# acproject/wsi-segmentation-pipeline

Hardware: AMD Instinct MI355X
Metric: patches/sec (256×256×3) whole-slide inference, 1/2/4/8 MI355X + CPU ref (higher is better)
Workload: dtype fp16 + MX-fp6 cross terms (fp32 accumulate); 1 GPU; cfg3: ONE 40000x40000 synthetic slide, tile 256 stride 256 -> 24648 tiles sharded over 1 rank(s) (each holds only its own slide regions: 4.80 GB on rank 0), ResNet-18 trunk + Classifier, fused read+normalise+conv HIP path, 1 all-gather, float64 stitch + softmax; tiles_total=24648, batch=6200, mode=mx, parallelism=tile-shard x1 + 1 all-gather, batches_in_flight=2

## Files before the change

include/wsi_hip.h:

```cpp
#ifndef WSI_HIP_H
#define WSI_HIP_H
#include <stddef.h>
#include <stdint.h>

#ifdef __cplusplus
extern "C" {
#endif

#define WSI_HIP_ABI_VERSION 9
int wsi_hip_abi_version(void);

size_t wsi_pf_bytes(int n, int h, int w, int c, int planes);
long long wsi_pf_pixel_index(int n, int y, int x, int h, int w);

size_t wsi_prepack_conv_bytes(int cout, int cin, int k, int planes);
int wsi_prepack_conv(const float* w, const float* bn_weight, const float* bn_bias, const float* bn_mean,
                     const float* bn_var, float eps, int cout, int cin, int k, int planes, void* wpk_out,
                     float* bias_out);
size_t wsi_prepack_stem_bytes(int planes);
int wsi_prepack_stem(const float* w, const float* bn_weight, const float* bn_bias, const float* bn_mean,
                     const float* bn_var, float eps, int planes, void* wpk_out, float* bias_out);
int wsi_prepack_stem_u8(const float* w, const float* bn_weight, const float* bn_bias, const float* bn_mean,
                        const float* bn_var, float eps, const float mean[3], const float std_[3], int planes,
                        void* wpk_out, float* bias_out);
// ... 14 lines not shown

enum {
    WSI_STEM_MODE_UNFUSED = 0,
    WSI_STEM_MODE_FUSED = 1,
    WSI_STEM_MODE_FUSED_LUT = 2,
    WSI_STEM_MODE_FUSED_ONE_STRIP = 3,
    WSI_STEM_MODE_FUSED_STRIPS = 4
};
int wsi_stem_set_mode(int fused, int rows_per_seg);

int wsi_conv3x3_bn_act(const void* in_pf, void* out_pf, const void* resid_pf, const void* wpk, const float* bias,
                       int n, int h_in, int w_in, int cin, int cout, int stride, int relu, int planes,
                       void* stream);
int wsi_conv1x1_bn(const void* in_pf, void* out_pf, const void* wpk, const float* bias, int n, int h_in, int w_in,
                   int cin, int cout, int stride, int planes, void* stream);
int wsi_conv1x1_bn_act(const void* in_pf, void* out_pf, const void* resid_pf, const void* wpk, const float* bias,
                       int n, int h_in, int w_in, int cin, int cout, int stride, int relu, int planes, void* stream);
int wsi_conv3x3_up_concat_bn_act(const void* up_pf, const void* skip_pf, void* out_pf, const void* wpk, const float* bias, int n, int h, int w,
                                 int c_up, int c_skip, int cout, int relu, int planes, void* stream);
int wsi_conv3x3s2_ds_fused(const void* in_pf, void* out_conv_pf, void* out_ds_pf, const void* wpk3, const float* bias3,
                           const void* wpk1, const float* bias1, int n, int h_in, int w_in, int cin, int cout, int planes,
                           void* stream);
int wsi_s2_slab_images(int n, int h_in, int w_in, int cin, int planes);
size_t wsi_pf_split_bytes(int n, int h, int w, int c, int planes);
int wsi_conv3x3_bn_act_split(const void* in_pf, void* out_split, const void* resid_pf, const void* wpk, const float* bias,
                             int n, int h, int w, int cin, int cout, int relu, int planes, void* stream);
int wsi_conv3x3s2_ds_fused_split(const void* in_split, void* out_conv_pf, void* out_ds_pf, const void* wpk3,
                                 const float* bias3, const void* wpk1, const float* bias1, int n, int h_in, int w_in,
                                 int cin, int cout, int planes, void* stream);
enum {
    WSI_CONV_MODE_S2_GATHER = 0,
    WSI_CONV_MODE_S2_SLAB = 1,
    WSI_CONV_MODE_S2_SLAB_128 = 3,
    WSI_CONV_MODE_XCD_ORDER = 8,
    WSI_CONV_MODE_WIDE_FROM_256 = 16,
    WSI_CONV_MODE_WIDE_NEVER = 32,
    WSI_CONV_MODE_S2_ABLATE = 64,
    WSI_CONV_MODE_NO_S2_SPLIT = 128,
    WSI_CONV_MODE_XCD_RANGES_OFF = 256,
    WSI_CONV_MODE_XCD_RANGES_L1 = 512,
    WSI_CONV_MODE_L1_SLAB3 = 1024,
    WSI_CONV_MODE_NO_DS_FOLD = 2048,
    WSI_CONV_MODE_NO_SLAB_PAIR = 4096,
    WSI_CONV_MODE_EPILOGUE_PIECES = 8192,
    WSI_CONV_MODE_L1_LINES128 = 16384,
    WSI_CONV_MODE_S2_NT2 = 32768,
    WSI_CONV_MODE_UNET_CONCAT_PASS = 65536,
    WSI_CONV_MODE_WIDE_NO_D8 = 131072,
    WSI_CONV_MODE_PW_GATHER = 262144,
    WSI_CONV_MODE_L1_PERSISTENT = 1048576,
    WSI_CONV_MODE_UNET_NO_TAIL = 2097152,
    WSI_CONV_MODE_UNET_TAIL_FORM1 = 4194304,
    WSI_CONV_MODE_UNET_X0_UNFUSED = 8388608,
    WSI_CONV_MODE_LINKNET_NO_TAIL = 16777216
};
int wsi_conv_set_mode(int mode);
int wsi_conv3x3_bn_act_cfg(const void* in_pf, void* out_pf, const void* resid_pf, const void* wpk, const float* bias,
                           int n, int h_in, int w_in, int cin, int cout, int stride, int relu, int planes, int cfg,
                           void* stream);

int wsi_avgpool_fc(const void* in_pf, int n, int h, int w, int c, const float* fc_w, const float* fc_b, int k,
                   float* feat_out, float* logits_out, int planes, void* stream);
int wsi_linear(const float* x, const float* w, const float* bias, float* y, int b, int k, int j, int relu,
               void* stream);

int wsi_pf_pack(const float* in_nchw, void* out_pf, int n, int c, int h, int w, int planes, void* stream);
int wsi_pf_unpack(const void* in_pf, float* out_nchw, int n, int c, int h, int w, int planes, void* stream);

#define WSI_TRUNK_MAX_BLOCKS 36
typedef struct {
    const void* stem_w;   const float* stem_b;
    const void* stem_w_u8; const float* stem_b_u8;
    float norm[6];
    int blocks[4];
    const void* conv_w[2 * WSI_TRUNK_MAX_BLOCKS]; const float* conv_b[2 * WSI_TRUNK_MAX_BLOCKS];
    const void* down_w[3];  const float* down_b[3];
    const float* head_w;  const float* head_b;  int head_k;
    int planes;
} wsi_trunk_weights;

size_t wsi_trunk_workspace_bytes(int n, int h, int w, int planes);
int wsi_trunk_workspace_init(void* workspace, int n, int h, int w, int planes, void* stream);
int wsi_trunk_workspace_release(void* workspace);
int wsi_trunk_forward(const wsi_trunk_weights* wt, const float* in_f32, const uint8_t* slide,
                      long long slide_pitch_bytes, int slide_h, int slide_w, const int* tile_xy, const float* lut,
                      int n, int h, int w, void* workspace, int workspace_n, float* feat_out ,
                      float* logits_out , float* fmap_out ,
                      void* stream);
int wsi_trunk_set_chunks(int stem_chunk, int layer1_chunk);
int wsi_trunk_forward_tap(const wsi_trunk_weights* wt, const float* in_f32, const uint8_t* slide,
                          long long slide_pitch_bytes, int slide_h, int slide_w, const int* tile_xy, const float* lut,
                          int n, int h, int w, void* workspace, int workspace_n, int stop_after, float* tap_out_nchw,
                          void* stream);

typedef struct {
    const void* stem_w;   const float* stem_b;
    const void* stem_w_u8; const float* stem_b_u8;
    float norm[6];
    int blocks[4];
    const void* conv_w[3 * WSI_TRUNK_MAX_BLOCKS]; const float* conv_b[3 * WSI_TRUNK_MAX_BLOCKS];
    const void* down_w[4];  const float* down_b[4];
    const float* head_w;  const float* head_b;  int head_k;
    int planes;
} wsi_bneck_weights;
size_t wsi_bneck_workspace_bytes(int n, int h, int w, int planes);
int wsi_bneck_workspace_init(void* workspace, int n, int h, int w, int planes, void* stream);
// ... 304 lines not shown
```

wsi_segmentation_pipeline_amd/csrc/capi.hip:

```cpp
#include "internal.h"
#include "edt_dev.h"
#include "regions_dev.h"
#include "../../include/wsi_hip.h"

ConvRoutes g_routes;

StemArgs stem_args(const TileSource& src, const void* wpk, const float* bias, float* scratch, int n, int h, int w) {
    StemArgs a;
    a.mode = src.in_f32 ? 0 : 1;
    a.in_f32 = src.in_f32; a.slide = src.slide; a.slide_pitch = src.pitch; a.SH = src.SH; a.SW = src.SW;
    a.origins = src.tile_xy; a.lut = src.lut; a.wpk = wpk; a.bias = bias; a.out = scratch;
    a.N = n; a.H = h; a.W = w; a.wpk_u8 = nullptr; a.bias_u8 = nullptr;
    return a;
}

int stem_run(const TileSource& src, const void* stem_wpk, const float* stem_bias, const void* stem_wpk_u8, const float* stem_bias_u8,
             const float* norm_mean_std, int n, int h, int w, float* scratch, void* out_pf, int planes, void* stream, int out96,
             long long plane96, void* x0_pf) {
    if (!stem_wpk || !stem_bias || !scratch || !out_pf || n <= 0 || h % 16 || w % 4) return WSI_EINVAL;
    if (!src.valid()) return WSI_EINVAL;
    StemArgs a = stem_args(src, stem_wpk, stem_bias, scratch, n, h, w);
    if (stem_wpk_u8 && stem_bias_u8 && norm_mean_std && !src.in_f32 && g_routes.stem_u8x) { a.wpk_u8 = stem_wpk_u8; a.bias_u8 = stem_bias_u8; }
    if (out96 && planes != 3) return WSI_EINVAL;
    if (x0_pf && !(a.wpk_u8 && g_routes.stem_fused && planes == 2)) return WSI_EINVAL;
// ... 201 lines not shown
int wsi_conv3x3s2_ds_fused(const void* in_pf, void* out_conv_pf, void* out_ds_pf, const void* wpk3, const float* bias3,
                           const void* wpk1, const float* bias1, int n, int h_in, int w_in, int cin, int cout, int planes,
                           void* stream) {
    if (!s2_ds_ok(in_pf, out_conv_pf, out_ds_pf, wpk3, bias3, wpk1, bias1, n, h_in, w_in, false)) return WSI_EINVAL;
    ConvArgs a = s2_ds_args(in_pf, out_conv_pf, out_ds_pf, wpk3, bias3, wpk1, bias1, n, h_in, w_in, cin, cout);
    const int per = wsi_s2_slab_images(n, h_in, w_in, cin, planes);
    const size_t bpc = planes == 1 ? PFmt<1>::BPC : PFmt<2>::BPC;
    const size_t in_img = (size_t)(h_in + 1) * (w_in + 1) * cin * bpc, out_img = (size_t)(h_in / 2 + 1) * (w_in / 2 + 1) * cout * bpc;
    int rc = WSI_EINVAL;
    for (int n0 = 0; per > 0 && n0 < n; n0 += per) {
        const int nn = n - n0 < per ? n - n0 : per;
        a.in = (const char*)in_pf + n0 * in_img;
        a.out = (char*)out_conv_pf + n0 * out_img;
        a.out2 = (char*)out_ds_pf + n0 * out_img;
        a.gi = pf_geom_fd(nn, h_in, w_in, cin);
        a.go = pf_geom_fd(nn, h_in / 2, w_in / 2, cout);
        rc = wsi_s2_dispatch(a, planes, (hipStream_t)stream);
        if (rc) break;
    }
    if (rc == WSI_EINVAL) {
        ConvCall c = {.in = in_pf, .out = out_conv_pf, .wpk = wpk3, .bias = bias3, .n = n, .h = h_in, .w = w_in, .cin = cin, .cout = cout,
                      .stride = 2, .ksize = 3, .relu = 1, .planes = planes, .stream = stream, .cfg = 0};
        rc = conv_common(c);
        c.out = out_ds_pf; c.wpk = wpk1; c.bias = bias1; c.ksize = 1; c.relu = 0;
        if (!rc) rc = conv_common(c);
    }
    return rc;
}

int wsi_conv_set_mode(int mode) {
    ConvRoutes& r = g_routes;
    const int base = mode & 7;
    r.s2_slab = base != WSI_CONV_MODE_S2_GATHER;
    r.s2_small_tiles = base != WSI_CONV_MODE_S2_SLAB_128;
    r.xcd_order = (mode & WSI_CONV_MODE_XCD_ORDER) ? 1 : 0;
    r.wide_min_c = (mode & WSI_CONV_MODE_WIDE_FROM_256) ? 256 : (mode & WSI_CONV_MODE_WIDE_NEVER) ? (1 << 30) : 128;
    r.s2_ablate = (mode & WSI_CONV_MODE_S2_ABLATE) ? 1 : 0;
    r.s2_split = (mode & WSI_CONV_MODE_NO_S2_SPLIT) ? 0 : 1;
    r.xcd_ranges = (mode & WSI_CONV_MODE_XCD_RANGES_OFF) ? 0 : (mode & WSI_CONV_MODE_XCD_RANGES_L1) ? 1 : 2;
    r.l1_rows = (mode & WSI_CONV_MODE_L1_SLAB3) ? 0 : 1;
    r.ds_fold = (mode & WSI_CONV_MODE_NO_DS_FOLD) ? 0 : 1;
    r.slab_pair = (mode & WSI_CONV_MODE_NO_SLAB_PAIR) ? 0 : 1;
    r.l1_lines96 = (mode & WSI_CONV_MODE_L1_LINES128) ? 0 : 1;
    r.s2_nt4 = (mode & WSI_CONV_MODE_S2_NT2) ? 0 : 1;
    r.unet_fuse_up = (mode & WSI_CONV_MODE_UNET_CONCAT_PASS) ? 0 : 1;
    r.wide_d8 = (mode & WSI_CONV_MODE_WIDE_NO_D8) ? 0 : 1;
    r.l1p = (mode & WSI_CONV_MODE_L1_PERSISTENT) ? 1 : 0;
    r.unet_tail = (mode & WSI_CONV_MODE_UNET_NO_TAIL) ? 0 : 1;
    r.unet_tail_form = (mode & WSI_CONV_MODE_UNET_TAIL_FORM1) ? 1 : 2;
    r.unet_x0_fused = (mode & WSI_CONV_MODE_UNET_X0_UNFUSED) ? 0 : 1;
    r.pw_gather = (mode & WSI_CONV_MODE_PW_GATHER) ? 1 : 0;
    r.linknet_tail = (mode & WSI_CONV_MODE_LINKNET_NO_TAIL) ? 0 : 1;
    r.epi_sectors = (mode & WSI_CONV_MODE_EPILOGUE_PIECES) ? 0 : 1;
    return WSI_OK;
}

int wsi_conv1x1_bn(const void* in_pf, void* out_pf, const void* wpk, const float* bias, int n, int h_in, int w_in,
                   int cin, int cout, int stride, int planes, void* stream) {
    return conv_common({.in = in_pf, .out = out_pf, .wpk = wpk, .bias = bias, .n = n, .h = h_in, .w = w_in, .cin = cin, .cout = cout,
                        .stride = stride, .ksize = 1, .relu = 0, .planes = planes, .stream = stream});
}

int wsi_conv1x1_bn_act(const void* in_pf, void* out_pf, const void* resid_pf, const void* wpk, const float* bias,
                       int n, int h_in, int w_in, int cin, int cout, int stride, int relu, int planes, void* stream) {
    return conv1x1_common({.in = in_pf, .out = out_pf, .resid = resid_pf, .wpk = wpk, .bias = bias, .n = n, .h = h_in, .w = w_in, .cin = cin,
                           .cout = cout, .stride = stride, .ksize = 1, .relu = relu, .planes = planes, .stream = stream});
}

int wsi_conv1x1_bn_relu_add(const void* in_pf, void* out_pf, const void* skip_pf, const void* wpk, const float* bias,
                            int n, int h, int w, int cin, int cout, int planes, void* stream) {
    if (!skip_pf) return WSI_EINVAL;
    return conv1x1_common({.in = in_pf, .out = out_pf, .resid = skip_pf, .wpk = wpk, .bias = bias, .n = n, .h = h, .w = w, .cin = cin,
                           .cout = cout, .stride = 1, .ksize = 1, .relu = 1, .planes = planes, .stream = stream, .resid_post = 1});
}

int wsi_tconv4x4s2_bn_relu(const void* in_pf, void* out_pf, const void* wpk, const float* bias, int n, int h, int w, int c, int planes,
                           void* stream) {
    if (!in_pf || !out_pf || !wpk || !bias || in_pf == out_pf || n <= 0 || h <= 0 || w <= 0 || c <= 0) return WSI_EINVAL;
    ConvArgs a = conv_args({.in = in_pf, .out = out_pf, .wpk = wpk, .bias = bias, .n = n, .h = h, .w = w, .cin = c, .cout = c, .stride = 1,
                            .ksize = 4, .relu = 1});
    a.go = pf_geom_fd(n, 2 * h, 2 * w, c);
    return wsi_tconv_dispatch(a, planes, (hipStream_t)stream);
}

int wsi_avgpool_fc(const void* in_pf, int n, int h, int w, int c, const float* fc_w, const float* fc_b, int k,
                   float* feat_out, float* logits_out, int planes, void* stream) {
    if (!in_pf || n <= 0 || (logits_out && (!fc_w || !fc_b || k <= 0))) return WSI_EINVAL;
    return wsi_avgpool_fc_dispatch(in_pf, pf_geom(n, h, w, c), fc_w, fc_b, k, feat_out, logits_out, planes,
                                   (hipStream_t)stream);
}

int wsi_linear(const float* x, const float* w, const float* bias, float* y, int b, int k, int j, int relu,
               void* stream) {
    if (!x || !w || !y) return WSI_EINVAL;
    return wsi_linear_dispatch(x, w, bias, y, b, k, j, relu, (hipStream_t)stream);
}

int wsi_pf_pack(const float* in_nchw, void* out_pf, int n, int c, int h, int w, int planes, void* stream) {
    if (!in_nchw || !out_pf || n <= 0 || planes < 1 || planes > 3 || c % (planes == 1 ? 64 : 32)) return WSI_EINVAL;
    return wsi_pf_pack_dispatch(in_nchw, out_pf, pf_geom(n, h, w, c), planes, (hipStream_t)stream);
}

int wsi_pf_unpack(const void* in_pf, float* out_nchw, int n, int c, int h, int w, int planes, void* stream) {
    if (!in_pf || !out_nchw || n <= 0 || planes < 1 || planes > 3 || c % (planes == 1 ? 64 : 32)) return WSI_EINVAL;
    return wsi_pf_unpack_dispatch(in_pf, out_nchw, pf_geom(n, h, w, c), planes, (hipStream_t)stream);
}
// ... 261 lines not shown
```

wsi_segmentation_pipeline_amd/csrc/common.h:

```cpp
#pragma once
#include <hip/hip_runtime.h>
#include <stdint.h>

typedef __attribute__((ext_vector_type(8))) __bf16 bf16x8;
typedef __attribute__((ext_vector_type(4))) __bf16 bf16x4;
typedef __attribute__((ext_vector_type(16))) float f32x16;
typedef __attribute__((ext_vector_type(4))) float f32x4;

#define WSI_OK 0
#define WSI_EINVAL (-22)
#define WSI_ENOMEM (-12)
#define WSI_EFAULT (-14)

struct FastDiv { unsigned m; int s; };
static inline FastDiv fastdiv_make(int d) {
    FastDiv f;
    if (d <= 1) { f.m = 0u; f.s = -1; return f; }
    int l = 0;
    while ((1ll << l) < d) ++l;
    f.m = (unsigned)(((1ull << (31 + l)) / (unsigned long long)d) + 1ull);
    f.s = l - 1;
    return f;
}
#ifdef __HIPCC__
// ... 19 lines not shown
    g.dHW = fastdiv_make(h * w); g.dW = fastdiv_make(w); g.dS = fastdiv_make(g.S); g.dP = fastdiv_make(g.P);
    return g;
}
static inline __device__ int pf_pos_of_index(const PFGeom& g, int i) {
    const int n = fd_div(i, g.dHW), rem = i - n * (g.H * g.W);
    const int y = fd_div(rem, g.dW), x = rem - y * g.W;
    return g.G + n * g.S + y * g.P + x;
}

#define PF_TILE_ROUND 512

static inline __host__ __device__ long long pf_alloc_pixels(int n, int h, int w) {
    long long P = w + 1, S = (long long)(h + 1) * P, G = P + 1;
    long long body = ((long long)n * S + PF_TILE_ROUND - 1) / PF_TILE_ROUND * PF_TILE_ROUND;
    return 2 * G + body + PF_TILE_ROUND;
}

static inline __device__ bool pf_is_pixel(const PFGeom& g, int q) {
    int r = q - g.G;
    if (r < 0 || r >= g.NS) return false;
    int x = r % g.P;
    int y = (r / g.P) % (g.H + 1);
    return x != g.W && y != g.H;
}

template <int PLANES> struct PFmt {
    static constexpr int BPC = PLANES == 1 ? 2 : 4;
    static constexpr int CPL = PLANES == 1 ? 64 : 32;
};
typedef __attribute__((ext_vector_type(8))) _Float16 f16x8;
typedef __attribute__((ext_vector_type(4))) _Float16 f16x4;
typedef __attribute__((ext_vector_type(8))) int i32x8;
typedef __attribute__((ext_vector_type(4))) unsigned int u32x4;
typedef __attribute__((ext_vector_type(2))) float f32x2;
typedef __attribute__((ext_vector_type(2))) _Float16 f16x2;
typedef __attribute__((ext_vector_type(4))) int i32x4;

struct ConvArgs {
    const void* in;
    void* out;
    const void* resid;
    const void* wpk;
    const float* bias;
    PFGeom gi, go;
    int stride;
    int ksize;
    int relu;
    int flags;
    void* out2;
    const void* wpk2;
    const float* bias2;
    long long out_split_pixels, in_split_pixels;
    int mtiles = 0;
    const void* in2 = nullptr;
    int in2_c = 0;
    const void* in_up = nullptr;
    int up_c = 0;
    PFGeom gup = {};
    long long plane96 = 0;
};

enum : int {
    CONV_XCD_ORDER = 1,
    CONV_XCD_RANGES = 2,
    CONV_RESID_DIRECT = 4,
    CONV_IN96 = 16, CONV_OUT96 = 32, CONV_RESID96 = 64,
    CONV_RESID_POST = 128,
    CONV_ABL_NO_STORE = 1 << 8, CONV_ABL_DISPATCH_ONLY = 1 << 9, CONV_ABL_NO_MAINLOOP = 1 << 10, CONV_NONTEMPORAL = 1 << 11,
    CONV_STORE_SECTORS = 1 << 12,
    CONV_WCOPIES_SHIFT = 16,
};
#ifdef WSI_STUDY
#define CONV_STUDY(a, bits) ((a).flags & (bits))
#else
#define CONV_STUDY(a, bits) 0
#endif

static inline __device__ size_t pf_out_offset(const PFGeom& g, long long split_pixels, int q, size_t pixstride) {
    if (!split_pixels) return (size_t)q * pixstride;
    int r = q - g.G;
    const int n = fd_div(r, g.dS);
    r -= n * g.S;
    const int y = fd_div(r, g.dP), x = r - y * g.P;
    const int P2 = g.W / 2 + 1, S2 = (g.H / 2 + 1) * P2;
    const long long q2 = (long long)(P2 + 1) + (long long)n * S2 + (y >> 1) * P2 + (x >> 1);
    return (size_t)(((y & 1) * 2 + (x & 1)) * split_pixels + q2) * pixstride;
}

static inline __device__ f32x16 mfma_bf16(bf16x8 a, bf16x8 b, f32x16 c) {
    return __builtin_amdgcn_mfma_f32_32x32x16_bf16(a, b, c, 0, 0, 0);
}
template <int PLANES> struct PairElem { typedef __bf16 T; };
template <> struct PairElem<2> { typedef _Float16 T; };
template <int PLANES>
static inline __device__ f32x16 mfma16(bf16x8 a, bf16x8 b, f32x16 c) {
    typedef __attribute__((ext_vector_type(8))) _Float16 h8;
    if constexpr (PLANES == 2) return __builtin_amdgcn_mfma_f32_32x32x16_f16(__builtin_bit_cast(h8, a), __builtin_bit_cast(h8, b), c, 0, 0, 0);
    else return __builtin_amdgcn_mfma_f32_32x32x16_bf16(a, b, c, 0, 0, 0);
}

typedef __attribute__((ext_vector_type(6))) unsigned u32x6;
typedef __attribute__((ext_vector_type(16))) unsigned u32x16;
typedef __attribute__((ext_vector_type(32))) float f32x32;
static inline __host__ __device__ int mx6_scale_byte(float amax) {
    union { float f; unsigned u; } c;
    c.f = amax;
// ... 102 lines not shown
}
static inline __device__ const float* conv_wscale_inv(const void* wpk, int cout, int cin, int ksize) {
    return (const float*)((const char*)wpk + (size_t)(cout / 32) * (cin / 32) * ksize * ksize * 4096);
}

constexpr int STEM_I8_DIGITS = 3;
constexpr int STEM_I8_SCALE_OFFSET = 2 * 7 * STEM_I8_DIGITS * 1024;
struct StemArgs {
    int mode;
    const float* in_f32;
    const uint8_t* slide;
    long long slide_pitch;
    int SH, SW;
    const int* origins;
    const float* lut;
    const void* wpk;
    const float* bias;
    float* out;
    int N, H, W;
    const void* wpk_u8;
    const float* bias_u8;
    void* out_pf = nullptr;
    int out_planes = 0;
};

struct ConvRoutes {
    int stem_fused = 1;
    int stem_rows = 64;
    int stem_u8x = 1;
    int stem_shared_weights = 1;
    int stem_dense = 1;
    int chunk_stem = 0;
    int chunk_l1 = 0;
    int s2_slab = 1;
    int s2_small_tiles = 1;
    int xcd_order = 0;
    int wide_min_c = 128;
    int s2_ablate = 0;
    int s2_split = 1;
    int xcd_ranges = 2;
    int l1_rows = 1;
    int ds_fold = 1;
    int slab_pair = 1;
    int l1_lines96 = 1;
    int s2_nt4 = 1;
    int unet_fuse_up = 1;
    int wide_d8 = 1;
    int l1p = 0;
    int unet_tail = 1;
    int unet_tail_form = 2;
    int unet_x0_fused = 1;
    int pw_gather = 0;
    int linknet_tail = 1;
    int epi_sectors = 1;
};
extern ConvRoutes g_routes;
```

wsi_segmentation_pipeline_amd/csrc/conv.hip:

```cpp
#include "conv_dev.h"
#include "internal.h"

template <int MT, int WM, int WN, int PLANES, bool POST = false>
__global__ __launch_bounds__(WM* WN * 64) void conv_gather_kernel(ConvArgs a) {
    extern __shared__ __attribute__((aligned(16))) char smem[];
    constexpr int BM = WM * MT * 32;
    constexpr int NTHREADS = WM * WN * 64;
    constexpr int PPT = BM * 8 / NTHREADS;
    constexpr int PIX_STEP = NTHREADS / 8;
    const int tid = threadIdx.x, lane = tid & 63, wave = tid >> 6;
    const int wm = wave / WN, wn = wave % WN;
    const int l31 = lane & 31, h = lane >> 5;
    const int nblocks = a.go.C / (WN * 32);
    const int nb = blockIdx.x % nblocks;
    const int mtile = blockIdx.x / nblocks;
    const int q0 = a.go.G + mtile * BM;
    const int ntile = nb * WN + wn;
    const int NC = a.gi.C / PFmt<PLANES>::CPL;
    const int KS = a.ksize, NT = KS * KS, pad = KS / 2;
    const size_t in_pixstride = (size_t)a.gi.C * PFmt<PLANES>::BPC;
    const bf16x8* wbase = (const bf16x8*)a.wpk + (size_t)ntile * NC * NT * 4 * 64 + lane;

    int inq[PPT];
    const int sp = tid & 7;
// ... 941 lines not shown
        asm volatile("s_waitcnt vmcnt(0)" ::: "memory");
        __syncthreads();
        xload(xf[0], xoff[0] + tap_off(0, Pc));
#pragma unroll
        for (int t = 0; t < NT; ++t) {
            asm volatile("" ::: "memory");
            if constexpr (!(ABL & 16)) {
                if (t + 1 < NT) wload(wbuf[(t + 1) % RING], c, t + 1);
                else if (c + 1 < NC) wload(wbuf[0], c + 1, 0);
            }
            asm volatile("" ::: "memory");
            const int toff = tap_off(t, Pc);
            const int toff_next = t + 1 < NT ? tap_off(t + 1, Pc) : 0;
#pragma unroll
            for (int mt = 0; mt < MT; ++mt) {
                const int k = t * MT + mt;
                if (mt + 1 < MT) xload(xf[(k + 1) & 1], xoff[mt + 1] + toff);
                else if (t + 1 < NT) xload(xf[(k + 1) & 1], xoff[0] + toff_next);
                const bf16x8(&w)[4] = wbuf[t % RING];
                const bf16x8(&x)[4] = xf[k & 1];
                f32x16& d = (FUSE && t == 9) ? accd[FUSE ? mt : 0] : acc[mt];
                if constexpr (PLANES == 3) {
                    d = mfma_mx6(d, w, x);
                } else if constexpr (PLANES == 2) {
                    mfma_step<2>(d, w, x);
                } else {
#pragma unroll
                    for (int f = 0; f < 4; ++f) d = mfma_bf16(w[f], x[f], d);
                }
            }
        }
    }
    conv_epilogue_any<MT, PLANES>(a, acc, q0 + wm * MT * 32, ntile, lane);
    if constexpr (FUSE) {
        ConvArgs a2 = a;
        a2.out = a.out2; a2.bias = a.bias2; a2.resid = nullptr; a2.relu = 0;
        a2.wpk = a.wpk2; a2.ksize = 1;
        conv_epilogue_any<MT, PLANES>(a2, accd, q0 + wm * MT * 32, ntile, lane);
    }
}

template <int MT, int WM, int WN, int PLANES, int MINW, bool FUSE, int PMAX = 34, int ABL = 0>
static int launch_s2slab(const ConvArgs& a, hipStream_t st) {
    constexpr int BM = WM * MT * 32, NTHREADS = WM * WN * 64;
    if (a.go.C % (WN * 32) || a.go.P > PMAX) return WSI_EINVAL;
    if ((unsigned long long)pf_alloc_pixels(a.gi.N, a.gi.H, a.gi.W) * a.gi.C * PFmt<PLANES>::BPC >= 0xffffffffull) return WSI_EINVAL;
    const int mtiles = (a.go.NS + BM - 1) / BM;
    const int nblocks = a.go.C / (WN * 32);
    const size_t lds = conv_slab_lds(4 * BM + 2 * a.go.P + 2, NTHREADS, 0);
    if (lds > 160 * 1024) return WSI_EINVAL;
    return conv_launch(conv3x3s2_slab_kernel<MT, WM, WN, PLANES, MINW, FUSE, PMAX, ABL>, conv_grid(mtiles, nblocks, a.flags & CONV_XCD_ORDER), NTHREADS, lds, st, a);
}

template <int PLANES, bool DENSE, bool DS, int NT = 2>
__global__ __launch_bounds__(512, 1) void conv3x3s2_wide_kernel(ConvArgs a) {
    extern __shared__ __attribute__((aligned(16))) char smem[];
    static_assert(NT == 2 || (NT == 4 && !DS), "four channel tiles per wave: no second accumulator set");
    constexpr int MT = 2, BM = 256, NTILES = 2 * NT, ULEN = NT == 2 ? 2 : 1;
    constexpr int WBUF = NTILES * 4096, XB = 45056;
    constexpr int NWB = 2 * ULEN;
    char* const wl = smem;
    char* const xl0 = smem + NWB * WBUF;
    const int tid = threadIdx.x, lane = tid & 63;
    const int wave = __builtin_amdgcn_readfirstlane(tid >> 6);
    const int wm = wave >> 1, wn = wave & 1;
    const int l31 = lane & 31, h = lane >> 5;
    const int nblocks = a.go.C / (NTILES * 32);
    int nb, mtile;
    if (!conv_tile_of_block(CONV_XCD_RANGES, nblocks, a.mtiles, nb, mtile)) return;
    const int P = a.go.P;
    int q0, qlast, qs[MT];
    bool valid[MT];
    if constexpr (!DENSE) {
        q0 = a.go.G + mtile * BM;
        qlast = q0 + BM - 1;
#pragma unroll
        for (int mt = 0; mt < MT; ++mt) {
            qs[mt] = q0 + wm * MT * 32 + mt * 32 + l31;
            valid[mt] = pf_is_pixel(a.go, qs[mt]);
        }
    } else {
        const int HW = a.go.H * a.go.W, R = a.go.N * HW;
        auto pos = [&](int i) { return pf_pos_of_index(a.go, i); };
        const int i0 = mtile * BM, i1 = min(i0 + BM, R) - 1;
        q0 = pos(i0);
        qlast = pos(i1);
#pragma unroll
        for (int mt = 0; mt < MT; ++mt) {
            const int i = i0 + wm * MT * 32 + mt * 32 + (a.go.W < 32 ? dense_lane_pixel(l31) : l31);
            valid[mt] = i < R;
            qs[mt] = pos(valid[mt] ? i : i1);
        }
    }
    const int NC = a.gi.C / PFmt<PLANES>::CPL;
    const size_t in_pixstride = (size_t)a.gi.C * PFmt<PLANES>::BPC;
    const __amdgpu_buffer_rsrc_t wrs = __builtin_amdgcn_make_buffer_rsrc(
        (void*)((const char*)a.wpk + (size_t)(nb * NTILES) * NC * 9 * 4096), 0, NTILES * NC * 9 * 4096, 0x00020000);
    const __amdgpu_buffer_rsrc_t wrd = __builtin_amdgcn_make_buffer_rsrc(
        (void*)((const char*)(DS ? a.wpk2 : a.wpk) + (size_t)(nb * NTILES) * NC * 4096), 0, NTILES * NC * 4096, 0x00020000);
    const int wvoff = lane * 16;
    auto wdma = [&](int c, int t, char* wb) {
#pragma unroll
        for (int j = 0; j < NTILES; ++j) {
            if (t < 9) dma16_buf_asm(wrs, lds_addr_of(wb) + j * 4096 + (wave - 4) * 1024, wvoff, ((j * NC + c) * 9 + t) * 4096 + (wave - 4) * 1024);
            else dma16_buf_asm(wrd, lds_addr_of(wb) + j * 4096 + (wave - 4) * 1024, wvoff, (j * NC + c) * 4096 + (wave - 4) * 1024);
        }
    };
    auto xdma = [&](int c, int ph, char* xb) {
        const int back = ((ph & 2) ? P : 0) + (ph & 1);
        const char* src = (const char*)a.in + ((size_t)ph * a.in_split_pixels + (size_t)(q0 - back)) * in_pixstride + c * 128;
        const int npieces = (qlast - q0 + 1 + back) * 8;
        for (int i0 = wave * 64; i0 < npieces; i0 += 256) {
            const int i = i0 + lane;
            dma16_asm(src + (size_t)(i >> 3) * in_pixstride + slab_lane_slot(i) * 16, lds_addr_of(xb) + i0 * 16);
        }
    };
    auto wread = [&](bf16x8(&w)[NT][4], const char* wb) {
        const char* src = wb + (wn * NT) * 4096 + lane * 16;
#pragma unroll
        for (int nt = 0; nt < NT; ++nt) {
#pragma unroll
            for (int f = 0; f < 4; ++f) w[nt][f] = *(const bf16x8*)(src + nt * 4096 + f * 1024);
        }
    };

    f32x16 acc[NT][MT], accd[DS ? NT : 1][DS ? MT : 1];
#pragma unroll
    for (int nt = 0; nt < NT; ++nt) {
        conv_acc_start<PLANES, MT>(acc[nt], a.bias, nb * NTILES + wn * NT + nt, lane);
        if constexpr (DS) conv_acc_start<PLANES, MT>(accd[nt], a.bias2, nb * NTILES + wn * NT + nt, lane);
    }

    constexpr int SPL = DS ? 10 : 9;
    constexpr int STEP_TAP[10] = {4, DS ? 9 : 3, DS ? 3 : 5, DS ? 5 : 1, DS ? 1 : 7, DS ? 7 : 0, DS ? 0 : 2, DS ? 2 : 6, DS ? 6 : 8, 8};
    constexpr int UNIT0[4] = {0, DS ? 2 : 1, DS ? 4 : 3, DS ? 6 : 5};
    constexpr int NSTEP[4] = {DS ? 2 : 1, 2, 2, 4};
    const int NG = NC * SPL;
    auto wdma_step = [&](int c, int j) {
        const int cc = c + j / SPL, g = cc * SPL + j % SPL;
        if (g < NG) wdma(cc, STEP_TAP[j % SPL], wl + (g & (NWB - 1)) * WBUF);
    };
    if (wave < 4) xdma(0, 0, xl0);
    else { wdma_step(0, 0); if (NSTEP[0] == 2 && ULEN == 2) wdma_step(0, 1); }
    asm volatile("s_waitcnt vmcnt(0)" ::: "memory");
    __syncthreads();
    for (int c = 0; c < NC; ++c) {
#pragma unroll
        for (int ph = 0; ph < 4; ++ph) {
            const char* xl = xl0 + (size_t)(ph & 1) * XB;
            if (wave < 4) {
                if (ph < 3) xdma(c, ph + 1, xl0 + (size_t)((ph + 1) & 1) * XB);
                else if (c + 1 < NC) xdma(c + 1, 0, xl0);
            }
#pragma unroll
            for (int kp = 0; kp < NSTEP[ph]; kp += ULEN) {
                const int j0 = UNIT0[ph] + kp;
                const int ulen = NSTEP[ph] - kp >= ULEN ? ULEN : 1;
                const int jn = j0 + ulen;
                const int nlen = ULEN == 1 ? 1 : (kp + 2 < NSTEP[ph]) ? 2 : (ph < 3 ? (NSTEP[ph + 1] >= 2 ? 2 : 1) : (NSTEP[0] >= 2 ? 2 : 1));
                if (wave >= 4) { wdma_step(c, jn); if (nlen == 2) wdma_step(c, jn + 1); }
#pragma unroll
                for (int k = 0; k < ulen; ++k) {
                    const int g = c * SPL + j0 + k;
                    const int t = STEP_TAP[j0 + k];
                    constexpr bool PREF = NT == 2 && !DS;
                    bf16x8 wf[NT][4], xf[PREF ? 2 : MT][4];
                    wread(wf, wl + (g & (NWB - 1)) * WBUF);
                    const int sh = (t < 9 && t % 3 == 2 ? 1 : 0) + (t < 9 && t / 3 == 2 ? P : 0);
                    auto xload = [&](bf16x8(&x)[4], int mt) {
                        int ql = qs[mt] - q0;
                        asm volatile("" : "+v"(ql));
                        const int Pl = ql + sh;
                        const int base = lds_xbase(Pl, h);
#pragma unroll
                        for (int f = 0; f < 4; ++f) x[f] = *(const bf16x8*)(xl + (base ^ (f << 5)));
                    };
                    if constexpr (PREF) {
                        xload(xf[0], 0);
#pragma unroll
                        for (int mt = 0; mt < MT; ++mt) {
                            if (mt + 1 < MT) xload(xf[(mt + 1) & 1], mt + 1);
                            __builtin_amdgcn_sched_barrier(0);
#pragma unroll
                            for (int nt = 0; nt < NT; ++nt) mfma_step<PLANES>(acc[nt][mt], wf[nt], xf[mt & 1]);
                            __builtin_amdgcn_sched_barrier(0);
                        }
                    } else {
#pragma unroll
                        for (int mt = 0; mt < MT; ++mt) xload(xf[mt], mt);
#pragma unroll
                        for (int mt = 0; mt < MT; ++mt)
#pragma unroll
                            for (int nt = 0; nt < NT; ++nt) {
                                if constexpr (DS) mfma_step<PLANES>(t == 9 ? accd[nt][mt] : acc[nt][mt], wf[nt], xf[mt]);
                                else mfma_step<PLANES>(acc[nt][mt], wf[nt], xf[mt]);
                            }
                    }
                }
                if (wave >= 4 || kp + ULEN >= NSTEP[ph]) asm volatile("s_waitcnt vmcnt(0)" ::: "memory");
                __syncthreads();
            }
        }
    }
#pragma unroll
    for (int nt = 0; nt < NT; ++nt) {
        const int ntile = nb * NTILES + wn * NT + nt;
        if constexpr (PLANES == 3) {
            conv_epilogue_mx<MT>(a, acc[nt], qs, valid, ntile, lane);
        } else {
            conv_epilogue_q<MT, PLANES>(a, acc[nt], qs, valid, ntile, lane);
        }
        if constexpr (DS) {
            ConvArgs a2 = a;
            a2.out = a.out2; a2.bias = a.bias2; a2.resid = nullptr; a2.relu = 0;
            a2.wpk = a.wpk2; a2.ksize = 1;
            if constexpr (PLANES == 3) conv_epilogue_mx<MT>(a2, accd[nt], qs, valid, ntile, lane);
            else conv_epilogue_q<MT, PLANES>(a2, accd[nt], qs, valid, ntile, lane);
        }
    }
}

template <int PLANES>
static int launch_s2wide(const ConvArgs& a, hipStream_t st) {
    constexpr int BM = 256, XB = 45056;
    const bool ds = a.out2 != nullptr;
    if (a.go.C % 128 || a.go.P > 34 || !a.in_split_pixels || (ds && (!a.wpk2 || !a.bias2)) || a.out_split_pixels) return WSI_EINVAL;
    const long long R = (long long)a.go.N * a.go.H * a.go.W;
    const bool nt4 = !ds && PLANES == 3 && g_routes.s2_nt4 && a.go.C % 256 == 0;
    const int nblocks = a.go.C / (nt4 ? 256 : 128);
    ConvArgs g = a;
    g.gi = a.go;
    const long long span = dense_max_slab_pixels(g, BM) - (a.go.P + 1);
    const bool dense = (span * 8 + 255) / 256 * 256 * 16 <= XB;
    const int mtiles = dense ? (int)((R + BM - 1) / BM) : (a.go.NS + BM - 1) / BM;
    const size_t lds = 4 * 16384 + 2 * XB;
    auto k = nt4 ? (dense ? conv3x3s2_wide_kernel<PLANES, true, false, 4> : conv3x3s2_wide_kernel<PLANES, false, false, 4>)
           : dense ? (ds ? conv3x3s2_wide_kernel<PLANES, true, true> : conv3x3s2_wide_kernel<PLANES, true, false>)
                   : (ds ? conv3x3s2_wide_kernel<PLANES, false, true> : conv3x3s2_wide_kernel<PLANES, false, false>);
    ConvArgs b = a;
    b.mtiles = mtiles;
    return conv_launch(k, conv_grid(mtiles, nblocks, CONV_XCD_RANGES), 512, lds, st, b);
}

int wsi_s2_dispatch(const ConvArgs& a_in, int planes, hipStream_t st) {
    ConvArgs a = a_in;
    if (a.in_split_pixels)
        return by_planes<P23>(planes, [&](auto p) { return launch_s2wide<p()>(a, st); });
    if (g_routes.xcd_order && a.go.C > 128) a.flags |= CONV_XCD_ORDER;
    if (a.gi.C % 64 || a.go.C % 128 || planes < 1 || planes > 3) return WSI_EINVAL;
    if (a.go.H * 2 != a.gi.H || a.go.W * 2 != a.gi.W || a.gi.N != a.go.N) return WSI_EINVAL;
    const bool fuse = a.out2 != nullptr;
    if (fuse && (!a.wpk2 || !a.bias2)) return WSI_EINVAL;
    if (a.go.P > 34)
        return by_planes<P23>(planes, [&](auto p) { return fuse ? launch_s2slab<2, 1, 4, p(), 2, true, 130>(a, st) : launch_s2slab<2, 1, 4, p(), 2, false, 130>(a, st); });
#ifdef WSI_STUDY
    if (g_routes.s2_ablate && planes == 3 && fuse) return launch_s2slab<2, 1, 4, 3, 3, true, 34, 16>(a, st);
#endif
    if (g_routes.s2_small_tiles && planes >= 2)
        return by_planes<P23>(planes, [&](auto p) { return fuse ? launch_s2slab<2, 1, 4, p(), 3, true>(a, st) : launch_s2slab<2, 1, 4, p(), 3, false>(a, st); });
    return by_planes<P123>(planes, [&](auto p) { return fuse ? launch_s2slab<4, 1, 4, p(), 2, true>(a, st) : launch_s2slab<4, 1, 4, p(), 2, false>(a, st); });
}

template <int MT, int WM, int WN, int PLANES, bool POST = false>
static int launch_gather(const ConvArgs& a, hipStream_t st) {
    constexpr int BM = WM * MT * 32;
    if (a.go.C % (WN * 32)) return WSI_EINVAL;
    const int mtiles = (a.go.NS + BM - 1) / BM;
    const int nblocks = a.go.C / (WN * 32);
    return conv_launch(conv_gather_kernel<MT, WM, WN, PLANES, POST>, conv_grid(mtiles, nblocks, 0), WM * WN * 64, (size_t)BM * 128, st, a);
}

#define SLAB3_CFGS(X) \
    X(20, 4, 1, 4, 2, false) \
    X(21, 4, 2, 2, 2, false) \
    X(25, 2, 2, 4, 3, false) \
    X(27, 4, 4, 2, 1, false) \
    X(28, 2, 2, 2, 3, true) \
    X(29, 2, 2, 2, 4, true) \
    X(39, 4, 4, 2, 1, true) \
    X(26, 4, 1, 2, 3, false) \
    X(30, 4, 1, 4, 2, true) \
    X(31, 4, 2, 2, 2, true) \
    X(32, 2, 2, 4, 3, true) \
    X(33, 8, 1, 4, 2, true) \
    X(34, 8, 1, 2, 2, true) \
    X(35, 8, 2, 2, 2, true) \
    X(36, 4, 2, 4, 2, true) \
    X(37, 4, 1, 4, 3, true) \
    X(38, 4, 2, 2, 3, true)



int wsi_slab_dispatch_cfg(const ConvArgs& a_in, int planes, int cfg, hipStream_t st) {
// ... 86 lines not shown
```

wsi_segmentation_pipeline_amd/native.py:

```python
import contextlib
import ctypes as C
import enum
import os
import subprocess

_HERE = os.path.dirname(os.path.abspath(__file__))
LIB_PATH = os.path.join(_HERE, 'lib', 'libwsi_hip.so')
CSRC = os.path.join(_HERE, 'csrc')

_lib = None


class NativeLibraryMissing(RuntimeError):
    pass


TRUNK_MAX_BLOCKS = 36


def _trunk_weights(name, convs, downs, doc):
    fields = [
        ('stem_w', C.c_void_p), ('stem_b', C.c_void_p),
        ('stem_w_u8', C.c_void_p), ('stem_b_u8', C.c_void_p), ('norm', C.c_float * 6),
        ('blocks', C.c_int * 4),
# ... 247 lines not shown
    _lib = None
    return LIB_PATH


ABI_VERSION = 9


def load():
    global _lib
    if _lib is not None:
        return _lib
    if not os.path.exists(LIB_PATH):
        raise NativeLibraryMissing(
            '%s not found: the WSI inference path has no CPU fallback - build it first '
            '(python -c "import __graft_entry__ as g; g.build()" or make -C %s)' % (LIB_PATH, CSRC))
    lib = C.CDLL(LIB_PATH)
    for name, (res, args) in SIGNATURES.items():
        fn = getattr(lib, name)
        fn.restype = res
        fn.argtypes = args
    if lib.wsi_hip_abi_version() != ABI_VERSION:
        raise RuntimeError('libwsi_hip.so ABI version mismatch')
    if lib.wsi_jpeg_tables_bytes() != C.sizeof(WsiJpegTables) or lib.wsi_jpeg_tile_bytes() != C.sizeof(WsiJpegTile):
        raise RuntimeError('libwsi_hip.so wsi_jpeg_tables / wsi_jpeg_tile layout mismatch')
    _lib = lib
    return lib


class ConvMode(enum.IntFlag):
    S2_GATHER = 0
    S2_SLAB = 1
    S2_SLAB_128 = 3
    XCD_ORDER = 8
    WIDE_FROM_256 = 16
    WIDE_NEVER = 32
    S2_ABLATE = 64
    NO_S2_SPLIT = 128
    XCD_RANGES_OFF = 256
    XCD_RANGES_L1 = 512
    L1_SLAB3 = 1024
    NO_DS_FOLD = 2048
    NO_SLAB_PAIR = 4096
    EPILOGUE_PIECES = 8192
    L1_LINES128 = 16384
    S2_NT2 = 32768
    UNET_CONCAT_PASS = 65536
    WIDE_NO_D8 = 131072
    PW_GATHER = 262144
    L1_PERSISTENT = 1048576
    UNET_NO_TAIL = 2097152
    UNET_TAIL_FORM1 = 4194304
    UNET_X0_UNFUSED = 8388608
    LINKNET_NO_TAIL = 16777216


class StemMode(enum.IntEnum):
    UNFUSED = 0
    FUSED = 1
    FUSED_LUT = 2
    FUSED_ONE_STRIP = 3
    FUSED_STRIPS = 4


@contextlib.contextmanager
def conv_mode(flags=0, base=ConvMode.S2_SLAB):
    lib = load()
    check(lib.wsi_conv_set_mode(int(base) | int(flags)), 'wsi_conv_set_mode')
    try:
        yield
    finally:
        lib.wsi_conv_set_mode(int(ConvMode.S2_SLAB))


@contextlib.contextmanager
def stem_mode(fused, rows=64):
    lib = load()
    check(lib.wsi_stem_set_mode(int(fused), rows), 'wsi_stem_set_mode')
    try:
        yield
    finally:
        lib.wsi_stem_set_mode(int(StemMode.FUSED), 64)


def profiled(run, max_records=256, ms=False):
    lib = load()
    check(lib.wsi_prof_begin(max_records), 'wsi_prof_begin')
    try:
        out = run()
    finally:
        t, kind, flops = (C.c_float * max_records)(), (C.c_int * max_records)(), (C.c_double * max_records)()
        n = lib.wsi_prof_end(t, kind, flops, max_records)
    if not 0 <= n < max_records:
        raise RuntimeError('wsi_prof_end returned %d of at most %d records' % (n, max_records))
    return out, [(kind[i], flops[i]) + ((t[i],) if ms else ()) for i in range(n)]


def check(rc, what):
    if rc != 0:
        raise RuntimeError('%s failed with code %d (see include/wsi_hip.h error conventions)' % (what, rc))
```

Baseline: 125,800 patches/s.

## Triple-buffer pixel slabs and pipeline weight fragments in stride-2 wide conv

```diff
diff --git a/include/wsi_hip.h b/include/wsi_hip.h
--- a/include/wsi_hip.h
+++ b/include/wsi_hip.h
@@ -90,6 +90,8 @@
     WSI_CONV_MODE_UNET_NO_TAIL = 2097152,
     WSI_CONV_MODE_UNET_TAIL_FORM1 = 4194304,
     WSI_CONV_MODE_UNET_X0_UNFUSED = 8388608,
+    WSI_CONV_MODE_S2_RING2 = 33554432,
+    WSI_CONV_MODE_S2_FRAGS_UPFRONT = 67108864,
     WSI_CONV_MODE_LINKNET_NO_TAIL = 16777216
 };
 int wsi_conv_set_mode(int mode);
diff --git a/wsi_segmentation_pipeline_amd/csrc/capi.hip b/wsi_segmentation_pipeline_amd/csrc/capi.hip
--- a/wsi_segmentation_pipeline_amd/csrc/capi.hip
+++ b/wsi_segmentation_pipeline_amd/csrc/capi.hip
@@ -277,6 +277,8 @@
     r.pw_gather = (mode & WSI_CONV_MODE_PW_GATHER) ? 1 : 0;
     r.linknet_tail = (mode & WSI_CONV_MODE_LINKNET_NO_TAIL) ? 0 : 1;
     r.epi_sectors = (mode & WSI_CONV_MODE_EPILOGUE_PIECES) ? 0 : 1;
+    r.s2_ring3 = (mode & WSI_CONV_MODE_S2_RING2) ? 0 : 1;
+    r.s2_frag_pipe = (mode & WSI_CONV_MODE_S2_FRAGS_UPFRONT) ? 0 : 1;
     return WSI_OK;
 }
 
diff --git a/wsi_segmentation_pipeline_amd/csrc/common.h b/wsi_segmentation_pipeline_amd/csrc/common.h
--- a/wsi_segmentation_pipeline_amd/csrc/common.h
+++ b/wsi_segmentation_pipeline_amd/csrc/common.h
@@ -95,6 +95,7 @@
     const float* bias2;
     long long out_split_pixels, in_split_pixels;
     int mtiles = 0;
+    int s2_xb = 0;
     const void* in2 = nullptr;
     int in2_c = 0;
     const void* in_up = nullptr;
@@ -303,6 +304,8 @@
     int unet_x0_fused = 1;
     int pw_gather = 0;
     int linknet_tail = 1;
+    int s2_ring3 = 1;
+    int s2_frag_pipe = 1;
     int epi_sectors = 1;
 };
 extern ConvRoutes g_routes;
diff --git a/wsi_segmentation_pipeline_amd/csrc/conv.hip b/wsi_segmentation_pipeline_amd/csrc/conv.hip
--- a/wsi_segmentation_pipeline_amd/csrc/conv.hip
+++ b/wsi_segmentation_pipeline_amd/csrc/conv.hip
@@ -1017,15 +1017,19 @@
     return conv_launch(conv3x3s2_slab_kernel<MT, WM, WN, PLANES, MINW, FUSE, PMAX, ABL>, conv_grid(mtiles, nblocks, a.flags & CONV_XCD_ORDER), NTHREADS, lds, st, a);
 }
 
-template <int PLANES, bool DENSE, bool DS, int NT = 2>
+template <int PLANES, bool DENSE, bool DS, int NT = 2, bool RING3 = false, bool FPIPE = false>
 __global__ __launch_bounds__(512, 1) void conv3x3s2_wide_kernel(ConvArgs a) {
     extern __shared__ __attribute__((aligned(16))) char smem[];
     static_assert(NT == 2 || (NT == 4 && !DS), "four channel tiles per wave: no second accumulator set");
-    constexpr int MT = 2, BM = 256, NTILES = 2 * NT, ULEN = NT == 2 ? 2 : 1;
-    constexpr int WBUF = NTILES * 4096, XB = 45056;
+    static_assert(!RING3 || NT == 2, "three pixel buffers: 16 KB weight stages only");
+    static_assert(!FPIPE || NT == 4, "weight fragments one channel tile ahead: the four-tile form");
+    constexpr int MT = 2, BM = 256, NTILES = 2 * NT, ULEN = (NT == 2 && !RING3) ? 2 : 1;
+    constexpr int WBUF = NTILES * 4096;
+    const int XB = RING3 ? a.s2_xb : 45056;
     constexpr int NWB = 2 * ULEN;
     char* const wl = smem;
     char* const xl0 = smem + NWB * WBUF;
+    WSTAMP(const unsigned long long st_begin = __builtin_readcyclecounter(); unsigned long long st_pro = 0, st_line = 0, st_tap = 0, st_a = 0;)
     const int tid = threadIdx.x, lane = tid & 63;
     const int wave = __builtin_amdgcn_readfirstlane(tid >> 6);
     const int wm = wave >> 1, wn = wave & 1;
@@ -1105,17 +1109,45 @@
         const int cc = c + j / SPL, g = cc * SPL + j % SPL;
         if (g < NG) wdma(cc, STEP_TAP[j % SPL], wl + (g & (NWB - 1)) * WBUF);
     };
-    if (wave < 4) xdma(0, 0, xl0);
-    else { wdma_step(0, 0); if (NSTEP[0] == 2 && ULEN == 2) wdma_step(0, 1); }
-    asm volatile("s_waitcnt vmcnt(0)" ::: "memory");
+    auto xdma_count = [&](int ph) {
+        const int npieces = (qlast - q0 + 1 + ((ph & 2) ? P : 0) + (ph & 1)) * 8 - wave * 64;
+        return __builtin_amdgcn_readfirstlane(npieces > 0 ? (npieces + 255) >> 8 : 0);
+    };
+    auto vm_wait = [&](int n) {
+        switch (n) {
+#define WSI_VMW(N) case N: asm volatile("s_waitcnt vmcnt(" #N ")" ::: "memory"); break;
+            WSI_VMW(1) WSI_VMW(2) WSI_VMW(3) WSI_VMW(4) WSI_VMW(5) WSI_VMW(6) WSI_VMW(7) WSI_VMW(8) WSI_VMW(9) WSI_VMW(10) WSI_VMW(11)
+#undef WSI_VMW
+            default: asm volatile("s_waitcnt vmcnt(0)" ::: "memory"); break;
+        }
+    };
+    int xcnt[4] = {0, 0, 0, 0};
+    if constexpr (RING3) {
+#pragma unroll
+        for (int ph = 0; ph < 4; ++ph) xcnt[ph] = xdma_count(ph);
+    }
+    WSTAMP(const unsigned long long st_setup = __builtin_readcyclecounter();)
+    if (wave < 4) {
+        xdma(0, 0, xl0);
+        if constexpr (RING3) xdma(0, 1, xl0 + XB);
+    } else { wdma_step(0, 0); if (NSTEP[0] == 2 && ULEN == 2) wdma_step(0, 1); }
+    if (RING3 && wave < 4) vm_wait(xcnt[1]);
+    else asm volatile("s_waitcnt vmcnt(0)" ::: "memory");
     __syncthreads();
+    WSTAMP(st_pro = __builtin_readcyclecounter() - st_setup;)
+    int cm = 0;
     for (int c = 0; c < NC; ++c) {
 #pragma unroll
         for (int ph = 0; ph < 4; ++ph) {
-            const char* xl = xl0 + (size_t)(ph & 1) * XB;
+            const char* xl = xl0 + (size_t)(RING3 ? (cm + ph) % 3 : (ph & 1)) * XB;
             if (wave < 4) {
-                if (ph < 3) xdma(c, ph + 1, xl0 + (size_t)((ph + 1) & 1) * XB);
-                else if (c + 1 < NC) xdma(c + 1, 0, xl0);
+                if constexpr (RING3) {
+                    if (ph < 2) xdma(c, ph + 2, xl0 + (size_t)((cm + ph + 2) % 3) * XB);
+                    else if (c + 1 < NC) xdma(c + 1, ph - 2, xl0 + (size_t)((cm + ph + 2) % 3) * XB);
+                } else {
+                    if (ph < 3) xdma(c, ph + 1, xl0 + (size_t)((ph + 1) & 1) * XB);
+                    else if (c + 1 < NC) xdma(c + 1, 0, xl0);
+                }
             }
 #pragma unroll
             for (int kp = 0; kp < NSTEP[ph]; kp += ULEN) {
@@ -1129,8 +1161,13 @@
                     const int g = c * SPL + j0 + k;
                     const int t = STEP_TAP[j0 + k];
                     constexpr bool PREF = NT == 2 && !DS;
-                    bf16x8 wf[NT][4], xf[PREF ? 2 : MT][4];
-                    wread(wf, wl + (g & (NWB - 1)) * WBUF);
+                    bf16x8 wf[FPIPE ? 2 : NT][4], xf[PREF ? 2 : MT][4];
+                    const char* const wsrc = wl + (g & (NWB - 1)) * WBUF;
+                    auto wread1 = [&](bf16x8(&w)[4], int nt) {
+#pragma unroll
+                        for (int f = 0; f < 4; ++f) w[f] = *(const bf16x8*)(wsrc + (wn * NT + nt) * 4096 + lane * 16 + f * 1024);
+                    };
+                    if constexpr (!FPIPE) wread(wf, wsrc);
                     const int sh = (t < 9 && t % 3 == 2 ? 1 : 0) + (t < 9 && t / 3 == 2 ? P : 0);
                     auto xload = [&](bf16x8(&x)[4], int mt) {
                         int ql = qs[mt] - q0;
@@ -1150,6 +1187,20 @@
                             for (int nt = 0; nt < NT; ++nt) mfma_step<PLANES>(acc[nt][mt], wf[nt], xf[mt & 1]);
                             __builtin_amdgcn_sched_barrier(0);
                         }
+                    } else if constexpr (FPIPE) {
+#pragma unroll
+                        for (int mt = 0; mt < MT; ++mt) {
+                            xload(xf[mt], mt);
+                            if (mt == 0) wread1(wf[0], 0);
+                        }
+#pragma unroll
+                        for (int nt = 0; nt < NT; ++nt) {
+                            if (nt + 1 < NT) wread1(wf[(nt + 1) & 1], nt + 1);
+                            __builtin_amdgcn_sched_barrier(0);
+#pragma unroll
+                            for (int mt = 0; mt < MT; ++mt) mfma_step<PLANES>(acc[nt][mt], wf[nt & 1], xf[mt]);
+                            __builtin_amdgcn_sched_barrier(0);
+                        }
                     } else {
 #pragma unroll
                         for (int mt = 0; mt < MT; ++mt) xload(xf[mt], mt);
@@ -1162,11 +1213,18 @@
                             }
                     }
                 }
-                if (wave >= 4 || kp + ULEN >= NSTEP[ph]) asm volatile("s_waitcnt vmcnt(0)" ::: "memory");
+                WSTAMP(st_a = __builtin_readcyclecounter();)
+                if (RING3 && wave < 4) {
+                    if (kp + ULEN >= NSTEP[ph]) vm_wait(ph < 2 ? xcnt[ph + 2] : (c + 1 < NC ? xcnt[ph - 2] : 0));
+                } else if (wave >= 4 || kp + ULEN >= NSTEP[ph]) asm volatile("s_waitcnt vmcnt(0)" ::: "memory");
+                WSTAMP(if (wave < 4) { st_line += __builtin_readcyclecounter() - st_a; st_a = __builtin_readcyclecounter(); })
                 __syncthreads();
-            }
-        }
-    }
+                WSTAMP(st_tap += __builtin_readcyclecounter() - st_a;)
+            }
+        }
+        if constexpr (RING3) cm = cm == 2 ? 0 : cm + 1;
+    }
+    WSTAMP(const unsigned long long st_loop_end = __builtin_readcyclecounter();)
 #pragma unroll
     for (int nt = 0; nt < NT; ++nt) {
         const int ntile = nb * NTILES + wn * NT + nt;
@@ -1183,6 +1241,7 @@
             else conv_epilogue_q<MT, PLANES>(a2, accd[nt], qs, valid, ntile, lane);
         }
     }
+    WSTAMP(wide_stamps_report(lane, st_begin, st_setup, st_pro, st_line, st_tap, st_loop_end);)
 }
 
 template <int PLANES>
@@ -1198,12 +1257,21 @@
     const long long span = dense_max_slab_pixels(g, BM) - (a.go.P + 1);
     const bool dense = (span * 8 + 255) / 256 * 256 * 16 <= XB;
     const int mtiles = dense ? (int)((R + BM - 1) / BM) : (a.go.NS + BM - 1) / BM;
-    const size_t lds = 4 * 16384 + 2 * XB;
-    auto k = nt4 ? (dense ? conv3x3s2_wide_kernel<PLANES, true, false, 4> : conv3x3s2_wide_kernel<PLANES, false, false, 4>)
-           : dense ? (ds ? conv3x3s2_wide_kernel<PLANES, true, true> : conv3x3s2_wide_kernel<PLANES, true, false>)
-                   : (ds ? conv3x3s2_wide_kernel<PLANES, false, true> : conv3x3s2_wide_kernel<PLANES, false, false>);
+    const long long item = dense ? span : BM + a.go.P + 1;
+    const size_t xb3 = (size_t)((item * 8 + 63) / 64 * 1024);
+    const bool ring3 = g_routes.s2_ring3 && !nt4 && 2 * 16384 + 3 * xb3 <= 160 * 1024;
+    const bool fpipe = g_routes.s2_frag_pipe && nt4;
+    const size_t lds = ring3 ? 2 * 16384 + 3 * xb3 : 4 * 16384 + 2 * XB;
+    auto pick = [&](auto dn) {
+        constexpr bool D = decltype(dn)::value;
+        if (nt4) return fpipe ? conv3x3s2_wide_kernel<PLANES, D, false, 4, false, true> : conv3x3s2_wide_kernel<PLANES, D, false, 4>;
+        if (!ds) return ring3 ? conv3x3s2_wide_kernel<PLANES, D, false, 2, true> : conv3x3s2_wide_kernel<PLANES, D, false>;
+        return ring3 ? conv3x3s2_wide_kernel<PLANES, D, true, 2, true> : conv3x3s2_wide_kernel<PLANES, D, true>;
+    };
+    auto k = dense ? pick(std::true_type{}) : pick(std::false_type{});
     ConvArgs b = a;
     b.mtiles = mtiles;
+    b.s2_xb = (int)xb3;
     return conv_launch(k, conv_grid(mtiles, nblocks, CONV_XCD_RANGES), 512, lds, st, b);
 }
 
diff --git a/wsi_segmentation_pipeline_amd/native.py b/wsi_segmentation_pipeline_amd/native.py
--- a/wsi_segmentation_pipeline_amd/native.py
+++ b/wsi_segmentation_pipeline_amd/native.py
@@ -323,6 +323,8 @@
     UNET_TAIL_FORM1 = 4194304
     UNET_X0_UNFUSED = 8388608
     LINKNET_NO_TAIL = 16777216
+    S2_RING2 = 33554432
+    S2_FRAGS_UPFRONT = 67108864
 
 
 class StemMode(enum.IntEnum):
```

Result: no change. 126,300 patches/s, median of 6 (+0.4%).
